# WdBlink/pyflyt-drone

Measured on AMD Instinct MI355X. Metric: env-steps/sec at N parallel envs (FixedwingWaypoints), higher is better.
Workload: dtype f64

## Files before the change

pyflyt-drone_amd/csrc/fwsim.hip:

```cpp
#include <hip/hip_runtime.h>

#include <algorithm>
#include <cmath>
#include <cstdio>
#include <cstdlib>
#include <cstring>
#include <map>
#include <mutex>
#include <new>
#include <string>
#include <type_traits>
#include <vector>

#include "fwsim_device.hpp"
#include "fwsim_rollout.hpp"
#include "fwsim_ppo.hpp"
#include "fwsim_collect.hpp"
#include "fwsim_fused.hpp"
#include "fwsim_objlock.hpp"
#include "fwsim_render.hpp"

using namespace fwsim;


// ... 87 lines not shown
  int left = (fresh && !begin) ? min(total - done, max_chunk > 0 ? max_chunk : P.step_ratio) : 0;
  if (__ballot(begin || left > 0) == 0ull) return;
  const DevState<T> V = shadow_view<T>(D);
  if (begin) {
    Rigid<T> S0; int32_t tick0 = 0, episode = (int32_t)target - 1, nr = 0; T wb0[3], wa0[3], wph0;
    T tm0[3]; (void)begin_reset<T, G>(P, V, env, S0, tick0, episode, nr, wb0, wa0, wph0, tm0);
    if (HASOBJ) {
      ObjState<T> O0;
      obj_reset_state<T, OBJ>(O0);
      if (OBJ) obj_spawn<T, G>(P, OC, V, env, target, leader, O0); else comb_spawn<T, G>(P, OC, V, env, target, leader, O0);
      if (leader) obj_store<T, OBJ>(V, env, O0);
    }
    if (leader) { store_rigid<T>(V, env, S0); D.is[env] = 0; D.sdone[env] = pack_done(target, D.epoch, sampled); }
  }
  if (__ballot(left > 0) == 0ull) return;
  TickC<T> C; SurfC<T> mine; T wmask;
  load_tick_constants<T, G, false>(Pp, C, mine, wmask);
  Rigid<T> S;
  load_rigid<T>(V, envc, S);
  T R[9];
  rot_from_unit_quat<T>(S.q, R);
  int32_t tick = D.is[envc];
  T wb[3], wa[3], wph;
#pragma unroll
  for (int k = 0; k < 3; ++k) { wb[k] = V.r[(RF_WIND + k) * n + envc]; wa[k] = V.r[(RF_WIND + 3 + k) * n + envc]; }
  wph = V.r[(RF_WIND + 6) * n + envc];
  T gust[2];
  gust_init<T>(P, wph, tick, gust);
  ObjState<T> O;
  if (HASOBJ) { obj_load<T, OBJ>(V, envc, O); O.near_mask = 0u; O.near_n = 0; }
  const T cmd0[FW_NUM_ACTUATORS] = {(T)0, (T)0, (T)0, (T)0, (T)0, (T)0};
  LaneAct<T> LA; LA.cmd = (T)0; LA.a = (T)0;
  if (G == 8) lane_act_scatter<T>(S, LA);
  const int chunk = left;
  int steps = sampled ? left : 0;
#pragma unroll 1
  while (__ballot(steps > 0) != 0ull) {
    const bool stepped = steps > 0;
    if (stepped) {
      (void)aviary_step<T, true, G, HASOBJ>(P, C, OC, V, envc, O, S, R, cmd0, tick, (T)0, (T)0, wb, wa, gust, mine, wmask, LA);
      steps -= 1;
    }
    if (HASOBJ) obj_capture_step<T, G>(OC, V, stepped, envc, O, S, R, tick);
  }
  if (G == 8) lane_act_gather<T>(S, LA);
  if (chunk > 0 && done + chunk == total) {
    T nd = (T)0;
    if (OBJ) obj_compute_state<T>(O);
    else {
      T t0[3];
#pragma unroll
      for (int k = 0; k < 3; ++k) t0[k] = V.r[(size_t)(RF_TARGETS + k) * n + envc];
      nd = end_reset<T, G>(P, V, envc, (int32_t)target, S, t0);
      if (COMB) comb_compute_state<T>(OC, O, P.num_targets == 0);
    }
    if (leader) {
      const T a0[4] = {(T)0, (T)0, (T)0, (T)0};
      T* orow = D.sobs + (size_t)env * P.obs_dim;
      if (OBJ) obj_write_obs<T>(P, O, S, a0, [&](int k, T v) { orow[k] = v; });
      else if (COMB) comb_write_obs<T>(P, V, env, O, S, a0, 0, [&](int k, T v) { orow[k] = v; });
      else write_obs<T>(P, V, env, S, a0, 0, [&](int k, T v) { orow[k] = v; });
      V.r[RF_NEW_DIST * n + env] = nd;
    }
  }
  if (chunk > 0 && leader) {
    store_rigid<T>(V, env, S);
    D.is[env] = tick;
    if (HASOBJ) obj_store<T, OBJ>(V, env, O);
    D.sdone[env] = pack_done(target, D.epoch, done + chunk);
  }
}

template <typename T, int G>
__device__ __forceinline__ void scenario_worker(const Params<T>* __restrict__ Pp, DevState<T> D, int blk) {
  constexpr int EPW = kWave / G;
  const int lane = threadIdx.x, sub = (G == 1) ? 0 : (lane & (G - 1)), row = lane / G;
  const int env = blk * EPW + row;
  const bool active = env < D.n;
  const int envc = active ? env : D.n - 1;
  const unsigned long long req = D.sreq[envc], dn = D.sdone[envc];
  const uint32_t target = (uint32_t)(req >> 32);
  const bool fresh = active && (uint32_t)req != D.epoch && req != ~0ull;
  const bool begin = fresh && (uint32_t)(dn >> 32) != target;
  if (__ballot(begin) == 0ull) return;
  if (begin) {
    const Params<T>& P = *Pp;
    Scenario<T> sc;
    sample_scenario_inl<T, G>(Pp, D.rs, (size_t)D.npad, env, target, &sc);
    T* orow = D.sobs + (size_t)env * P.obs_dim;
    for (int k = sub; k < P.att_dim; k += G) orow[k] = Pp->warm_obs[k];
    if (G > 1) {
      if (sub < P.ctx) {
        T d[3] = {(T)0, (T)0, (T)0}, b[3] = {(T)0, (T)0, (T)0};
        if (sub < P.num_targets) {
#pragma unroll
          for (int k = 0; k < 3; ++k) d[k] = sc.t_mine[k] - P.warm[k];
          mtv(P.warm_R, d, b);
        }
#pragma unroll
        for (int k = 0; k < 3; ++k) orow[P.att_dim + 3 * sub + k] = b[k];
      }
      if (sub == 0) {
        T nd = (T)0;
        if (P.num_targets > 0) {
          const T dx = sc.t_mine[0] - P.warm[0], dy = sc.t_mine[1] - P.warm[1], dz = sc.t_mine[2] - P.warm[2];
          nd = M<T>::sqrt_(dx * dx + dy * dy + dz * dz);
        }
        D.rs[(size_t)RF_NEW_DIST * D.npad + env] = nd;
      }
    }
    if (sub == 0) D.sdone[env] = pack_done(target, D.epoch, 1);
  }
}

#ifdef FW_PROFILE
#define FWP_NOW() ((long long)__builtin_readcyclecounter())
#define FWP(...) __VA_ARGS__
constexpr int kProfSlots = 256, kProfWords = 12;
#ifdef FW_PROFILE_PHASES
constexpr bool getenv_ph = true;
#else
constexpr bool getenv_ph = false;
#endif
#else
#define FWP(...)
#endif

enum Phase : int { PH_STEP = 0, PH_WARM = 1, PH_DONE = 2 };

template <typename T, bool GENERAL, int G, int TKIND, int WPE = 1, bool COLLECT = false, bool HELP = false, bool AX = false, bool AUX = false,
          typename SH = ShapeOfParams>
__device__ __forceinline__
void step_body(const Params<T>* __restrict__ Pp, const ObjC<T>* __restrict__ OCp, DevState<T> Dg,
               const T* __restrict__ actions, T* __restrict__ obs, T* __restrict__ reward,
               uint8_t* __restrict__ terminated, uint8_t* __restrict__ truncated, T* __restrict__ terminal_obs,
               int32_t* __restrict__ info, const CollectArgs* __restrict__ CAp = nullptr) {
  extern __shared__ __align__(16) unsigned char smem_raw[];
  T* tile = reinterpret_cast<T*>(smem_raw);
  const Params<T>& P = *Pp;
  constexpr bool OBJ = TKIND == FW_TASK_OBJLOCK;
  constexpr bool COMB = TKIND == FW_TASK_WAYPOINT_OBJLOCK;
  constexpr bool HASOBJ = OBJ || COMB;
  constexpr int EPW = kWave / G;
  constexpr bool DEFER = !GENERAL && TKIND == FW_TASK_WAYPOINTS;
  static_assert(!SH::kFixed || (std::is_same<T, double>::value && DEFER && G == 8 && !COLLECT && !HELP), "a fixed shape is threaded through the wind-free 8-lane waypoints path only");
  const int nblk = (Dg.npad + EPW - 1) / EPW;
  FWP(const long long p_t0 = FWP_NOW(); long long p_reset = 0, p_avi = 0, p_task = 0, p_r1 = 0, p_r2 = 0, p_r3 = 0; int p_nreset = 0, p_nhit = 0;)
  const int bx = (int)blockIdx.x - (COLLECT ? CAp->n_act : 0);
  const int wg = SH::kFixed ? (bx >= nblk ? bx - nblk : bx) : bx % nblk;
  const int blk = (G == 8 && (nblk & 7) == 0) ? (wg & 7) * (nblk >> 3) + (wg >> 3) : wg;
  const DevState<T> D = tile_view<T, EPW>(Dg, blk);
  if ((GENERAL || DEFER) && bx >= nblk) {
    if (AUX && threadIdx.x >= kWave) return;
    DevState<T> Dw = D;
    if constexpr (SH::kFixed) Dw.epoch = launch_index(Dg.lctr);
    if (GENERAL) shadow_worker<T, G, TKIND>(Pp, OCp, Dw, blk); else scenario_worker<T, G>(Pp, Dw, blk);
    FWP(if (D.prof && threadIdx.x == 0) {
      long long* w = D.prof + ((size_t)(Dw.epoch % kProfSlots) * 2 * nblk + blockIdx.x) * kProfWords;
      w[0] = FWP_NOW() - p_t0; })
    if constexpr (SH::kFixed) launch_done(Dg.lctr, Dw.epoch);
    return;
  }
  const int lane = AUX ? (int)(threadIdx.x & (kWave - 1)) : (int)threadIdx.x;
  const int sub = (G == 1) ? 0 : (lane & (G - 1));
  const int row = lane / G;
  const bool leader = sub == 0;
  const int env0 = blk * EPW;
  const int env = env0 + row;
  const bool active = env < D.n;
  const int envc = active ? env : D.n - 1;
  const size_t n = D.npad;
  const int Dobs = FW_SH(obs_dim);
  const int ld = Dobs + 1;

  T* aux_nz = AUX ? reinterpret_cast<T*>(smem_raw + Dg.mbox_off) : nullptr;
  if constexpr (AUX) {
    if (threadIdx.x >= kWave) {
      const int32_t a_tick = D.i[IF_TICK * n + envc], a_episode = D.i[IF_EPISODE * n + envc], a_flags = D.i[IF_FLAGS * n + envc];
      T a_z0 = (T)0, a_z1 = (T)0;
      if (FW_SH(has_noise) && FW_SH(step_ratio) <= G && !(a_flags & (FL_TERM | FL_TRUNC)))
        rng_normal2<T>(P, (uint32_t)(P.env_offset + envc), (uint32_t)a_episode, (uint32_t)(a_tick / FW_SH(ticks_per_aviary)) + (uint32_t)sub, a_z0, a_z1);
      aux_nz[2 * lane] = a_z0; aux_nz[2 * lane + 1] = a_z1;
      __syncthreads();
      return;
    }
  }

  int32_t step_count = D.i[IF_STEP * n + envc];
  int32_t tick = D.i[IF_TICK * n + envc];
  int32_t episode = D.i[IF_EPISODE * n + envc];
  int32_t flags = D.i[IF_FLAGS * n + envc];
  int32_t num_reached = D.i[IF_NUM_REACHED * n + envc];
  constexpr bool LANE_T = DEFER && G == 8;
  T tmine[3] = {(T)0, (T)0, (T)0};
  T a_keep = (T)0;
  if (LANE_T) {
    if (sub < FW_SH(num_targets)) {
#pragma unroll
      for (int k = 0; k < 3; ++k) tmine[k] = D.r[(size_t)(RF_TARGETS + 3 * sub + k) * n + envc];
    }
    if (!COLLECT) a_keep = actions[(size_t)envc * 4 + (sub & 3)];
  }
  Rigid<T> S;
  load_rigid<T>(D, envc, S);
  T new_dist = D.r[RF_NEW_DIST * n + envc];
  T ep_return = D.r[RF_EP_RETURN * n + envc];
  TickC<T> C; SurfC<T> mine_regs; T wmask;
  if constexpr (SH::kFixed) load_step_image<T>(Pp, C, mine_regs, wmask);
  else load_tick_constants<T, G, DEFER && G == 8 && WPE == 1>(Pp, C, mine_regs, wmask);
  uint32_t lctr_v = 0;
  if constexpr (SH::kFixed) lctr_v = vload(Dg.lctr + blockIdx.x + opaque_zero());
  if (AX && !SH::kFixed && sub >= FW_NUM_SURFACES) mine_regs.hra = (T)0;
  SurfC<T>& mine = mine_regs;

  normalize_quat<T>(S.q);
  T R[9];
  rot_from_unit_quat<T>(S.q, R);
  ObjState<T> O;
  const ObjC<T>& OC = *OCp;
  if (HASOBJ) { obj_load<T, OBJ>(D, envc, O); obj_update_near_mask<T, G>(P, OC, D, envc, O, S); }
  int32_t out_strike = 0;
  unsigned long long sh_req = ~0ull, sh_done = 0ull;
  if ((GENERAL || DEFER) && D.shadow_on) { sh_req = D.sreq[envc]; sh_done = D.sdone[envc]; }
  T wb[3] = {(T)0, (T)0, (T)0}, wa[3] = {(T)0, (T)0, (T)0}, wphase = (T)0;
  if (GENERAL) {
#pragma unroll
    for (int k = 0; k < 3; ++k) { wb[k] = D.r[(RF_WIND + k) * n + envc]; wa[k] = D.r[(RF_WIND + 3 + k) * n + envc]; }
    wphase = D.r[(RF_WIND + 6) * n + envc];
  }
  T gust[2] = {(T)0, (T)1};
  if (GENERAL) gust_init<T>(P, wphase, tick, gust);
  T rew = (T)-0.1;
  T cmd[FW_NUM_ACTUATORS];
  double c_ret = 0.0;
  if (COLLECT) {
    if (active && leader) c_ret = ld_sc1(CAp->S.returns + env);
    collect_wait_actions(*CAp, Dg.epoch, env0, min(EPW, Dg.n - env0));
  }
  {
    const T* ap = actions + (size_t)envc * 4;
    T a4[4];
    if (COLLECT) collect_load_actions<T>(*CAp, ap, a4);
    else {
#pragma unroll
      for (int k = 0; k < 4; ++k) a4[k] = ap[k];
    }
    if (COLLECT && LANE_T) a_keep = (sub & 3) == 0 ? a4[0] : (sub & 3) == 1 ? a4[1] : (sub & 3) == 2 ? a4[2] : a4[3];
    const T sp[4] = { a4[0], a4[1], a4[2], a4[3] * (T)0.5 + (T)0.5 };
#pragma unroll
    for (int c = 0; c < FW_NUM_ACTUATORS; ++c)
      cmd[c] = P.mixer[c][0] * sp[0] + P.mixer[c][1] * sp[1] + P.mixer[c][2] * sp[2] + P.mixer[c][3] * sp[3];
  }
  LaneAct<T> LA; LA.a = (T)0; LA.cmd = (T)0;
  T cmd_mine = (T)0;
  if (G == 8) { lane_act_scatter<T>(S, LA); cmd_mine = lane_pick5<T>(cmd[0], cmd[1], cmd[2], cmd[3], cmd[4]); LA.cmd = cmd_mine; }

  T tcur[3] = {(T)0, (T)0, (T)0}, tnext[3] = {(T)0, (T)0, (T)0};
  const int gbase = lane & ~(G - 1);
  if (LANE_T) {
#pragma unroll
    for (int k = 0; k < 3; ++k) tcur[k] = __shfl(tmine[k], gbase | (num_reached & (G - 1)), kWave);
  } else if (!OBJ) {
    const int i0 = min(num_reached, FW_MAX_TARGETS - 1), i1 = min(num_reached + 1, FW_MAX_TARGETS - 1);
#pragma unroll
    for (int k = 0; k < 3; ++k) {
      tcur[k] = D.r[(size_t)(RF_TARGETS + 3 * i0 + k) * n + envc];
      tnext[k] = D.r[(size_t)(RF_TARGETS + 3 * i1 + k) * n + envc];
    }
  }

  const uint32_t genv = (uint32_t)(P.env_offset + envc);
  const bool done_at_entry = (flags & (FL_TERM | FL_TRUNC)) != 0;
  int tgt_obs = (flags >> FL_TGT_SHIFT) & 15;
  flags &= FL_MASK;
  int act_src = done_at_entry ? 1 : 0;

  const uint32_t astep0 = (uint32_t)(tick / FW_SH(ticks_per_aviary));
  const bool pre_noise = (G == 8) && FW_SH(has_noise) && (FW_SH(step_ratio) <= G);
  T nz0 = (T)0, nz1 = (T)0;
  if (!AUX && pre_noise && !done_at_entry) rng_normal2<T>(P, genv, (uint32_t)episode, astep0 + (uint32_t)sub, nz0, nz1);

  int phase = active ? PH_STEP : PH_DONE;
  constexpr bool STASH = (!DEFER && !HASOBJ) || COLLECT;
  double* latch = STASH ? reinterpret_cast<double*>(smem_raw + Dg.stash_off) : nullptr;
  int it = 0, warm_left = 0;
  const Mbox<T> MB = mbox_at<T>(HELP ? Dg.mbox_off : 0);
  uint32_t n_posted = 0, pend_seq = 0;
  int pend = 0;
  T dist_keep = (T)0;
  bool resetting = false;
  bool step_over = active && done_at_entry;
  int32_t k_max_steps = 0, k_auto_reset = 0; T k_dome = (T)0, k_reach = (T)0;
  if constexpr (SH::kFixed) {
    k_max_steps = P.max_steps; k_auto_reset = P.auto_reset; k_dome = P.dome; k_reach = P.reach;
    asm("" : "+s"(k_max_steps)); asm("" : "+s"(k_auto_reset)); asm("" : "+s"(k_dome)); asm("" : "+s"(k_reach));
  }
  if constexpr (SH::kFixed) asm volatile("" : "+v"(lctr_v));
  if constexpr (AUX) {
    __syncthreads();
    nz0 = aux_nz[2 * lane]; nz1 = aux_nz[2 * lane + 1];
  }

  FWP(const long long p_t1 = FWP_NOW();)
#pragma unroll 1
  for (;;) {
    FWP(const long long p_a = FWP_NOW();)
    if (phase == PH_STEP && step_over) {
      step_count += 1;
      ep_return += rew;
      phase = PH_DONE;
      if (STASH && leader) {
        latch[4 * row] = (double)rew; latch[4 * row + 1] = (flags & (FL_TERM | FL_TRUNC)) ? 1.0 : 0.0;
        latch[4 * row + 2] = __hiloint2double(num_reached, flags); latch[4 * row + 3] = __hiloint2double(out_strike, step_count);
      }
      if (!(STASH && !DEFER) && leader) {
        reward[env] = rew;
        terminated[env] = (uint8_t)((flags & FL_TERM) ? 1 : 0);
        truncated[env] = (uint8_t)((flags & FL_TRUNC) ? 1 : 0);
        if (info) {
          int4* ip = reinterpret_cast<int4*>(info + (size_t)env * FW_INFO_DIM);
          ip[0] = make_int4(num_reached, (flags & FL_COLLISION) ? 1 : 0, (flags & FL_OOB) ? 1 : 0, (flags & FL_COMPLETE) ? 1 : 0);
          ip[1] = make_int4(out_strike, OBJ ? out_strike : 0, step_count, 0);
        }
      }
      if (DEFER) { resetting = (flags & (FL_TERM | FL_TRUNC)) && (SH::kFixed ? k_auto_reset : P.auto_reset); FWP(if (resetting) p_nreset += 1;) }
      const bool take_shadow = GENERAL && (flags & (FL_TERM | FL_TRUNC)) && P.auto_reset && D.shadow_on &&
                               (int)(sh_done & 0xFF) == P.warmup_aviary_steps + 1 && (uint32_t)(sh_done >> 32) == (uint32_t)(episode + 1) &&
                               (uint32_t)((sh_done >> 8) & 0xFFFFFFu) != (D.epoch & 0xFFFFFFu);
      if (take_shadow) { resetting = true; FWP(p_nreset += 1; p_nhit += 1;) }
      if (!DEFER && !take_shadow && (flags & (FL_TERM | FL_TRUNC)) && P.auto_reset) {
        if (G == 8) lane_act_gather<T>(S, LA);
        if (terminal_obs && leader) {
          T* trow = terminal_obs + (size_t)env * Dobs;
          T act_t[4];
          load_action<T, COLLECT>(D, actions, env, act_src, act_t);
          if (OBJ) obj_write_obs<T>(P, O, S, act_t, [&](int k, T v) { trow[k] = v; });
          else if (COMB) comb_write_obs<T>(P, D, env, O, S, act_t, tgt_obs, [&](int k, T v) { trow[k] = v; });
          else write_obs<T>(P, D, env, S, act_t, tgt_obs, [&](int k, T v) { trow[k] = v; });
        }
        T t_mine[3] = {(T)0, (T)0, (T)0};
        FWP(const long long p_ra = FWP_NOW(); p_r1 += p_ra - p_a;)
        {
          if (leader) stat_add(D.stats, FW_CTR_FALLBACKS);
          warm_left = begin_reset<T, G>(P, D, env, S, tick, episode, num_reached, wb, wa, wphase, t_mine);
          if (G > 1) {
            const int src = lane & ~(G - 1);
#pragma unroll
            for (int k = 0; k < 3; ++k) t_mine[k] = __shfl(t_mine[k], src, kWave);
          }
          if (HASOBJ) {
            obj_reset_state<T, OBJ>(O);
            if (OBJ) obj_spawn<T, G>(P, OC, D, env, (uint32_t)episode, leader, O);
            else comb_spawn<T, G>(P, OC, D, env, (uint32_t)episode, leader, O);
          }
        }
        if (G > 1 && warm_left > 0) __builtin_amdgcn_fence(__ATOMIC_ACQ_REL, "workgroup");
        if (HASOBJ) obj_update_near_mask<T, G>(P, OC, D, env, O, S);
        if (GENERAL) gust_init<T>(P, wphase, tick, gust);
        if (G == 8) lane_act_scatter<T>(S, LA);
        FWP(const long long p_rb = FWP_NOW(); p_r2 += p_rb - p_ra;)
        step_count = 0; flags = 0; ep_return = (T)0; tgt_obs = 0;
        act_src = 2;
        if (leader) stat_add(D.stats, FW_CTR_RESETS);
        FWP(p_nreset += 1;)
        rot_from_unit_quat<T>(S.q, R);
        if (GENERAL && warm_left > 0) phase = PH_WARM;
        else if (OBJ) obj_compute_state<T>(O);
        else {
          new_dist = end_reset<T, G>(P, D, env, episode, S, t_mine);
          if (COMB) comb_compute_state<T>(OC, O, P.num_targets == 0);
        }
        FWP(p_r3 += FWP_NOW() - p_rb;)
      }
    }
    FWP(const long long p_b = FWP_NOW(); p_reset += p_b - p_a;)
    if (__ballot(phase != PH_DONE) == 0ull) break;
    T z0 = (T)0, z1 = (T)0;
    if (pre_noise) {
      const int src = (lane & ~(G - 1)) | (it & (G - 1));
      z0 = __shfl(nz0, src, kWave); z1 = __shfl(nz1, src, kWave);
    }
    const bool stepped = phase != PH_DONE;
    const bool stepping = stepped && (!GENERAL || phase == PH_STEP);
    bool contact = false;
    if (stepped) {
      if (FW_SH(has_noise) && !pre_noise && stepping)
        rng_normal2<T>(P, genv, (uint32_t)episode, (uint32_t)(tick / FW_SH(ticks_per_aviary)), z0, z1);
      if (GENERAL) {
        T c_eff[FW_NUM_ACTUATORS];
#pragma unroll
        for (int c = 0; c < FW_NUM_ACTUATORS; ++c) c_eff[c] = stepping ? cmd[c] : (T)0;
        z0 = stepping ? z0 : (T)0; z1 = stepping ? z1 : (T)0;
        LA.cmd = stepping ? cmd_mine : (T)0;
        contact = aviary_step<T, true, G, HASOBJ, AX, SH>(P, C, OC, D, env, O, S, R, c_eff, tick, z0, z1, wb, wa, gust, mine, wmask, LA);
      } else {
        contact = aviary_step<T, false, G, HASOBJ, AX, SH>(P, C, OC, D, env, O, S, R, cmd, tick, z0, z1, wb, wa, gust, mine, wmask, LA);
      }
    }
    if constexpr (HELP) {
      const bool due = stepped && OC.camera_ratio_ticks > 0 && (tick % OC.camera_ratio_ticks) == 0;
      FWP(const long long p_c0 = FWP_NOW(); p_avi += p_c0 - p_b;)
      const uint32_t seq_cur = cap_post<T>(MB, n_posted, due, row, leader, O, S, R);
      FWP(p_r1 += FWP_NOW() - p_c0;)
      FWP(const long long p_w0 = FWP_NOW();)
      cap_collect<T>(MB, pend_seq, (pend & 2) != 0, row, O, D.stats);
      FWP(p_task += FWP_NOW() - p_w0;)
      pend_seq = 0;
      auto frame_half = [&](int keep) {
        if (OBJ) {
          obj_compute_state<T>(O);
          if ((keep & 4) && obj_reward<T>(OC, P.sparse, O, dist_keep, rew)) { flags |= FL_TERM | FL_COMPLETE; out_strike = 1; }
        } else {
          comb_compute_state<T>(OC, O, (keep & 8) != 0);
          if (keep & 4) {
            if (!(keep & 8)) comb_obstacle_penalty<T>(OC, O, (T)1, rew);
            else {
              comb_obstacle_penalty<T>(OC, O, (T)0.5, rew);
              if (comb_duck_reward<T>(OC, P.sparse, O, rew)) { flags |= FL_TERM | FL_COMPLETE; out_strike = 1; }
            }
          }
        }
      };
      FWP(const long long p_f0 = FWP_NOW();)
      if (pend & 1) frame_half(pend);
      FWP(const long long p_f1 = FWP_NOW(); p_r2 += p_f1 - p_f0;)
      pend = 0;
      int keep = 0;
      bool now = false;
      if (stepped) {
        if (stepping) {
          keep = 1 | (due ? 2 : 0);
          int nleft = 0;
          T old_dist = new_dist;
          if (COMB) {
            nleft = P.num_targets - num_reached;
            if (nleft > 0) {
              T dx = tcur[0] - S.p[0], dy = tcur[1] - S.p[1], dz = tcur[2] - S.p[2];
              new_dist = M<T>::sqrt_(dx * dx + dy * dy + dz * dz);
            }
            tgt_obs = num_reached;
            if (nleft == 0) keep |= 8;
          }
          if (step_count > P.max_steps) flags |= FL_TRUNC;
          if (contact) { rew = (T)-100; flags |= FL_COLLISION | FL_TERM; }
          if (S.p[0] * S.p[0] + S.p[1] * S.p[1] + S.p[2] * S.p[2] > P.dome * P.dome) { rew = (T)-100; flags |= FL_OOB | FL_TERM; }
          bool can_strike = false;
          if (!(flags & (FL_COLLISION | FL_OOB))) {
            keep |= 4;
            if (OBJ) {
              T dx = O.duck[0] - S.p[0], dy = O.duck[1] - S.p[1], dz = O.duck[2] - S.p[2];
              dist_keep = M<T>::sqrt_(dx * dx + dy * dy + dz * dz);
              can_strike = O.lock_steps + (T)1 >= (T)OC.hold_steps && dist_keep <= OC.strike_dist;
            } else if (nleft > 0) {
              if (!P.sparse) {
                T progress = (old_dist != (T)0) ? (old_dist - new_dist) : (T)0;
                rew += M<T>::fmax_((T)3 * progress, (T)0);
                rew += M<T>::rcp_(new_dist);
              }
              if (new_dist < P.reach) {
                rew = (T)100;
                num_reached += 1;
                if (num_reached == P.num_targets) flags &= ~(FL_TERM | FL_TRUNC);
                const int i1 = min(num_reached + 1, FW_MAX_TARGETS - 1);
#pragma unroll
                for (int k = 0; k < 3; ++k) { tcur[k] = tnext[k]; tnext[k] = D.r[(size_t)(RF_TARGETS + 3 * i1 + k) * n + env]; }
              }
            } else {
              flags &= ~FL_TERM;
              can_strike = O.lock_steps + (T)1 >= (T)OC.hold_steps;
            }
          }
          step_over = (it + 1 >= P.step_ratio) || (flags & (FL_TERM | FL_TRUNC));
          now = can_strike || step_over;
        } else {
          now = true;
        }
      }
      auto finish_now = [&]() {
        if (stepping) {
          frame_half(keep);
          step_over = (it + 1 >= P.step_ratio) || (flags & (FL_TERM | FL_TRUNC));
        } else {
          warm_left -= 1;
          if (warm_left == 0) {
            if (OBJ) obj_compute_state<T>(O);
            else { new_dist = end_reset<T, G>(P, D, env, episode, S); comb_compute_state<T>(OC, O, P.num_targets == 0); }
            phase = PH_DONE;
          }
        }
      };
      FWP(const long long p_f2 = FWP_NOW(); p_r3 += p_f2 - p_f1;)
      bool wait_here;
      if constexpr (OBJ) wait_here = __ballot(now && due) != 0ull; else wait_here = __ballot(now) != 0ull;
      if (wait_here) {
        FWP(const long long p_w1 = FWP_NOW();)
        cap_collect<T>(MB, seq_cur, due, row, O, D.stats);
        FWP(p_task += FWP_NOW() - p_w1; p_nhit += 1;)
        FWP(const long long p_f3 = FWP_NOW();)
        if (stepped) finish_now();
        FWP(p_r2 += FWP_NOW() - p_f3;)
      } else {
        FWP(const long long p_f3 = FWP_NOW();)
        if constexpr (OBJ) { if (now) finish_now(); else pend = keep; }
        else pend = keep;
        FWP(p_r2 += FWP_NOW() - p_f3;)
        pend_seq = seq_cur;
      }
    } else {
    if (HASOBJ) obj_capture_step<T, G, COLLECT>(OC, D, stepped, envc, O, S, R, tick);
    FWP(const long long p_c = FWP_NOW(); p_avi += p_c - p_b;)
    if (stepped) {
      if (stepping && OBJ) {
        obj_compute_state<T>(O);
        if (step_count > P.max_steps) flags |= FL_TRUNC;
        if (contact) { rew = (T)-100; flags |= FL_COLLISION | FL_TERM; }
        if (S.p[0] * S.p[0] + S.p[1] * S.p[1] + S.p[2] * S.p[2] > P.dome * P.dome) { rew = (T)-100; flags |= FL_OOB | FL_TERM; }
        if (!(flags & (FL_COLLISION | FL_OOB))) {
          T dx = O.duck[0] - S.p[0], dy = O.duck[1] - S.p[1], dz = O.duck[2] - S.p[2];
          if (obj_reward<T>(OC, P.sparse, O, M<T>::sqrt_(dx * dx + dy * dy + dz * dz), rew)) {
            flags |= FL_TERM | FL_COMPLETE; out_strike = 1;
          }
        }
        step_over = (it + 1 >= P.step_ratio) || (flags & (FL_TERM | FL_TRUNC));
      } else if (stepping && COMB) {
        const int nleft = P.num_targets - num_reached;
        const T old_dist = new_dist;
        if (nleft > 0) {
          T dx = tcur[0] - S.p[0], dy = tcur[1] - S.p[1], dz = tcur[2] - S.p[2];
          new_dist = M<T>::sqrt_(dx * dx + dy * dy + dz * dz);
        }
        tgt_obs = num_reached;
        comb_compute_state<T>(OC, O, nleft == 0);
        if (step_count > P.max_steps) flags |= FL_TRUNC;
        if (contact) { rew = (T)-100; flags |= FL_COLLISION | FL_TERM; }
        if (S.p[0] * S.p[0] + S.p[1] * S.p[1] + S.p[2] * S.p[2] > P.dome * P.dome) { rew = (T)-100; flags |= FL_OOB | FL_TERM; }
        if (!(flags & (FL_COLLISION | FL_OOB))) {
          if (nleft > 0) {
            if (!P.sparse) {
              T progress = (old_dist != (T)0) ? (old_dist - new_dist) : (T)0;
              rew += M<T>::fmax_((T)3 * progress, (T)0);
              rew += M<T>::rcp_(new_dist);
            }
            if (new_dist < P.reach) {
              rew = (T)100;
              num_reached += 1;
              if (num_reached == P.num_targets) flags &= ~(FL_TERM | FL_TRUNC);
              const int i1 = min(num_reached + 1, FW_MAX_TARGETS - 1);
#pragma unroll
              for (int k = 0; k < 3; ++k) { tcur[k] = tnext[k]; tnext[k] = D.r[(size_t)(RF_TARGETS + 3 * i1 + k) * n + env]; }
            }
            comb_obstacle_penalty<T>(OC, O, (T)1, rew);
          } else {
            flags &= ~FL_TERM;
            comb_obstacle_penalty<T>(OC, O, (T)0.5, rew);
            if (comb_duck_reward<T>(OC, P.sparse, O, rew)) { flags |= FL_TERM | FL_COMPLETE; out_strike = 1; }
          }
        }
        step_over = (it + 1 >= P.step_ratio) || (flags & (FL_TERM | FL_TRUNC));
      } else if (stepping) {
        const int nleft = FW_SH(num_targets) - num_reached;
        const T old_dist = new_dist;
        if (FW_SH(task) != FW_TASK_OBJLOCK && nleft > 0) {
          T dx = tcur[0] - S.p[0], dy = tcur[1] - S.p[1], dz = tcur[2] - S.p[2];
          if constexpr (SH::kFixed) new_dist = M<T>::sqrt_(sum_squares_fma(dx, dy, dz));
          else new_dist = M<T>::sqrt_(dx * dx + dy * dy + dz * dz);
        }
        tgt_obs = num_reached;
        if (step_count > (SH::kFixed ? k_max_steps : P.max_steps)) flags |= FL_TRUNC;
        if (contact) { rew = (T)-100; flags |= FL_COLLISION | FL_TERM; }
        bool oob;
        if constexpr (SH::kFixed) oob = sum_squares_fma(S.p[0], S.p[1], S.p[2]) > k_dome * k_dome;
        else oob = S.p[0] * S.p[0] + S.p[1] * S.p[1] + S.p[2] * S.p[2] > P.dome * P.dome;
        if (oob) { rew = (T)-100; flags |= FL_OOB | FL_TERM; }
        if (FW_SH(task) != FW_TASK_OBJLOCK && nleft > 0) {
          if (!FW_SH(sparse)) {
            T progress = (old_dist != (T)0) ? (old_dist - new_dist) : (T)0;
            rew += M<T>::fmax_((T)3 * progress, (T)0);
            rew += M<T>::rcp_(new_dist);
          }
          if (new_dist < (SH::kFixed ? k_reach : P.reach)) {
            rew = (T)100;
            num_reached += 1;
            if (num_reached == FW_SH(num_targets)) flags |= FL_TRUNC | FL_COMPLETE;
            if (LANE_T) {
#pragma unroll
              for (int k = 0; k < 3; ++k) tcur[k] = __shfl(tmine[k], gbase | (num_reached & (G - 1)), kWave);
            } else {
              const int i1 = min(num_reached + 1, FW_MAX_TARGETS - 1);
#pragma unroll
              for (int k = 0; k < 3; ++k) { tcur[k] = tnext[k]; tnext[k] = D.r[(size_t)(RF_TARGETS + 3 * i1 + k) * n + env]; }
            }
          }
        }
        step_over = (it + 1 >= FW_SH(step_ratio)) || (flags & (FL_TERM | FL_TRUNC));
      } else {
        warm_left -= 1;
        if (warm_left == 0) {
          if (OBJ) obj_compute_state<T>(O);
          else { new_dist = end_reset<T, G>(P, D, env, episode, S); if (COMB) comb_compute_state<T>(OC, O, P.num_targets == 0); }
          phase = PH_DONE;
        }
      }
      FWP(p_task += FWP_NOW() - p_c;)
    }
    }
    it += 1;
  }
  FWP(const long long p_t2 = FWP_NOW();)
  if (G > 1 && !DEFER) __builtin_amdgcn_fence(__ATOMIC_ACQ_REL, "workgroup");
  if (G == 8) lane_act_gather<T>(S, LA);
  T tpre[3] = {(T)0, (T)0, (T)0};
  const uint32_t launch = SH::kFixed ? 1u + (uint32_t)__builtin_amdgcn_readfirstlane((int)lctr_v) : D.epoch;
  const bool pre = DEFER && resetting && D.shadow_on && (int)(sh_done & 0xFF) == 1 && (uint32_t)(sh_done >> 32) == (uint32_t)(episode + 1) &&
                   (uint32_t)((sh_done >> 8) & 0xFFFFFFu) != (launch & 0xFFFFFFu);
  if (pre) {
#pragma unroll
    for (int k = 0; k < 3; ++k) pf_issue(tpre[k], &D.rs[(size_t)(RF_TARGETS + 3 * sub + k) * n + env]);
  }
  constexpr bool WO = DEFER && G == 8;
  constexpr int kWO = WO ? 32 / G : 1;
  T wo[kWO];
  if (WO && resetting) {
#pragma unroll
    for (int j = 0; j < kWO; ++j) { const int k = sub + j * G; wo[j] = (k < FW_SH(att_dim)) ? vload(&Pp->warm_obs[k]) : (T)0; }
  }

  constexpr int kDOW = 4;
  T dow[kDOW], dnd = (T)0;
  if (WO && pre && Dobs <= kDOW * G) {
#pragma unroll
    for (int j = 0; j < kDOW; ++j) { const int k = sub + j * G; dow[j] = (T)0; if (k < Dobs) pf_issue(dow[j], &Dg.sobs[(size_t)env * Dobs + k]); }
    pf_issue(dnd, &D.rs[(size_t)RF_NEW_DIST * n + env]);
  }

  constexpr int kRows = HASOBJ ? RF_COUNT : RF_TASK;
  constexpr int kCW = GENERAL ? (kRows + G - 1) / G : 1, kOW = GENERAL ? (kMaxObs + G - 1) / G : 1;
  constexpr bool SWAP_REGS = GENERAL && G == 8;
  T cw[kCW], ow[kOW];
  int32_t tick_new = 0;
  constexpr bool PF_GEN = false;
  if (GENERAL && resetting) {
    if (SWAP_REGS) {
#pragma unroll
      for (int j = 0; j < kCW; ++j) {
        const int w = sub + j * G; cw[j] = (T)0;
        if (w < kRows) { if (PF_GEN) pf_issue(cw[j], &D.rs[(size_t)w * n + env]); else cw[j] = D.rs[(size_t)w * n + env]; }
      }
#pragma unroll
      for (int j = 0; j < kOW; ++j) {
        const int k = sub + j * G; ow[j] = (T)0;
        if (k < Dobs) { if (PF_GEN) pf_issue(ow[j], &Dg.sobs[(size_t)env * Dobs + k]); else ow[j] = Dg.sobs[(size_t)env * Dobs + k]; }
      }
    }
    tick_new = D.is[env];
  }
  const int ep_want = episode + 1 + ((GENERAL && resetting) ? 1 : 0);
  if ((GENERAL || DEFER) && D.shadow_on && active && leader && (uint32_t)(sh_req >> 32) != (uint32_t)ep_want)
    D.sreq[env] = ((unsigned long long)(uint32_t)ep_want << 32) | (unsigned long long)launch;
  T act_obs[4] = {(T)0, (T)0, (T)0, (T)0};
  if (LANE_T) {
#pragma unroll
    for (int k = 0; k < 4; ++k) act_obs[k] = __shfl(a_keep, gbase | k, kWave);
    if (act_src == 1) {
#pragma unroll
      for (int k = 0; k < 4; ++k) act_obs[k] = D.r[(size_t)(RF_ACTION + k) * n + envc];
    }
    T Ro[9];
    int o = write_obs_attitude<T, true, SH>(P, S, act_obs, Ro, [&](int k, T v) { if (leader) tile[row * ld + k] = v; });
#pragma unroll SH::kCtxUnroll
    for (int i = 0; i < FW_SH(ctx); ++i) {
      const int t = tgt_obs + i;
      T tw[3], d[3], b[3] = {(T)0, (T)0, (T)0};
#pragma unroll
      for (int k = 0; k < 3; ++k) tw[k] = __shfl(tmine[k], gbase | (t & (G - 1)), kWave);
      if (t < FW_SH(num_targets)) {
#pragma unroll
        for (int k = 0; k < 3; ++k) d[k] = tw[k] - S.p[k];
        mtv(Ro, d, b);
      }
      if (leader) { tile[row * ld + o] = b[0]; tile[row * ld + o + 1] = b[1]; tile[row * ld + o + 2] = b[2]; }
      o += 3;
    }
  } else if (active && leader) {
    load_action<T, COLLECT>(D, actions, env, act_src, act_obs);
    if (OBJ) obj_write_obs<T>(P, O, S, act_obs, [&](int k, T v) { tile[row * ld + k] = v; });
    else if (COMB) comb_write_obs<T>(P, D, env, O, S, act_obs, tgt_obs, [&](int k, T v) { tile[row * ld + k] = v; });
    else write_obs<T>(P, D, env, S, act_obs, tgt_obs, [&](int k, T v) { tile[row * ld + k] = v; });
  }
  FWP(const long long p_e0 = FWP_NOW();)
  if (DEFER && pre) {
    pf_wait(tpre[0], tpre[1], tpre[2], dnd);
    if (WO) pf_tie(dow[0], dow[1], dow[2], dow[3]);
  }
  if (DEFER && resetting) {
    __builtin_amdgcn_fence(__ATOMIC_ACQ_REL, "wavefront");
    if (terminal_obs) {
      T* trow = terminal_obs + (size_t)env * Dobs;
      for (int k = sub; k < Dobs; k += G) trow[k] = tile[row * ld + k];
    }
    __builtin_amdgcn_fence(__ATOMIC_ACQ_REL, "wavefront");
    FWP(const long long p_e1 = FWP_NOW(); p_r1 = p_e1 - p_e0;)
    episode += 1;
    if (leader) { stat_add(D.stats, FW_CTR_RESETS); stat_add(D.stats, pre ? FW_CTR_SCENARIO_HITS : FW_CTR_FALLBACKS); }
    Scenario<T> sc;
    if (pre) {
#pragma unroll
      for (int k = 0; k < 3; ++k) sc.t_mine[k] = tpre[k];
      if (sub < FW_SH(num_targets)) {
#pragma unroll
        for (int k = 0; k < 3; ++k) D.r[(size_t)(RF_TARGETS + 3 * sub + k) * n + env] = tpre[k];
      }
    } else {
      sample_scenario_inl<T, G>(Pp, D.r, n, env, (uint32_t)episode, &sc);
    }
    const int nt = min(FW_SH(ctx), FW_SH(num_targets));
    T t0[3] = {(T)0, (T)0, (T)0};
    const bool copied = WO && pre && Dobs <= kDOW * G;
    if (copied) {
#pragma unroll
      for (int j = 0; j < kDOW; ++j) { const int k = sub + j * G; if (k < Dobs) tile[row * ld + k] = dow[j]; }
    }
#pragma unroll 1
    for (int i = 0; i < (copied ? 0 : FW_SH(ctx)); ++i) {
      T tw[3] = {(T)0, (T)0, (T)0};
      if (G > 1) {
#pragma unroll
        for (int k = 0; k < 3; ++k) tw[k] = __shfl(sc.t_mine[k], (lane & ~(G - 1)) | (i & (G - 1)), kWave);
      } else if (i < nt) {
#pragma unroll
        for (int k = 0; k < 3; ++k) tw[k] = D.r[(size_t)(RF_TARGETS + 3 * i + k) * n + env];
      }
      T d[3] = {(T)0, (T)0, (T)0}, b[3] = {(T)0, (T)0, (T)0};
      if (i < nt) {
#pragma unroll
        for (int k = 0; k < 3; ++k) d[k] = tw[k] - P.warm[k];
        mtv(P.warm_R, d, b);
        if (i == 0) { t0[0] = tw[0]; t0[1] = tw[1]; t0[2] = tw[2]; }
      }
      if (leader) { tile[row * ld + FW_SH(att_dim) + 3 * i] = b[0]; tile[row * ld + FW_SH(att_dim) + 3 * i + 1] = b[1]; tile[row * ld + FW_SH(att_dim) + 3 * i + 2] = b[2]; }
    }
    FWP(const long long p_e2 = FWP_NOW(); p_r2 = p_e2 - p_e1;)
    if (WO && !copied) {
#pragma unroll
      for (int j = 0; j < kWO; ++j) { const int k = sub + j * G; if (k < FW_SH(att_dim)) tile[row * ld + k] = wo[j]; }
    }
    if (!copied) for (int k = sub + (WO ? kWO * G : 0); k < FW_SH(att_dim); k += G) tile[row * ld + k] = Pp->warm_obs[k];
#pragma unroll
    for (int k = 0; k < 3; ++k) { S.p[k] = P.warm[k]; S.v[k] = P.warm[7 + k]; S.w[k] = P.warm[10 + k]; }
#pragma unroll
    for (int k = 0; k < 4; ++k) S.q[k] = P.warm[3 + k];
#pragma unroll
    for (int k = 0; k < FW_NUM_ACTUATORS; ++k) S.act[k] = P.warm[13 + k];
    tick = P.warm_ticks;
    step_count = 0; flags = 0; ep_return = (T)0; tgt_obs = 0; num_reached = 0;
    new_dist = copied ? dnd : (T)0;
    if (FW_SH(num_targets) > 0 && !copied) {
      if (G == 1 && nt == 0) {
#pragma unroll
        for (int k = 0; k < 3; ++k) t0[k] = D.r[(size_t)(RF_TARGETS + k) * n + env];
      } else if (G > 1 && nt == 0) {
#pragma unroll
        for (int k = 0; k < 3; ++k) t0[k] = __shfl(sc.t_mine[k], lane & ~(G - 1), kWave);
      }
      T dx = t0[0] - S.p[0], dy = t0[1] - S.p[1], dz = t0[2] - S.p[2];
      new_dist = M<T>::sqrt_(dx * dx + dy * dy + dz * dz);
    }
#pragma unroll
    for (int k = 0; k < 4; ++k) act_obs[k] = (T)0;
    FWP(p_r3 = FWP_NOW() - p_e2;)
  }
  if (PF_GEN && resetting) {
    asm volatile("s_waitcnt vmcnt(0)" ::: "memory");
#pragma unroll
    for (int j = 0; j < kCW; ++j) asm volatile("" : "+v"(cw[j]));
#pragma unroll
    for (int j = 0; j < kOW; ++j) asm volatile("" : "+v"(ow[j]));
  }
  if (GENERAL && resetting) {
    __builtin_amdgcn_fence(__ATOMIC_ACQ_REL, "wavefront");
    if (terminal_obs) {
      T* trow = terminal_obs + (size_t)env * Dobs;
      for (int k = sub; k < Dobs; k += G) trow[k] = tile[row * ld + k];
    }
    __builtin_amdgcn_fence(__ATOMIC_ACQ_REL, "wavefront");
    if (SWAP_REGS) {
#pragma unroll
      for (int j = 0; j < kOW; ++j) { const int k = sub + j * G; if (k < Dobs) tile[row * ld + k] = ow[j]; }
#pragma unroll
      for (int j = 0; j < kCW; ++j) { const int w = sub + j * G; if (w < kRows) D.r[(size_t)w * n + env] = cw[j]; }
    } else {
      for (int k = 0; k < Dobs; ++k) tile[row * ld + k] = Dg.sobs[(size_t)env * Dobs + k];
      copy_words<T, G>(D.r, D.rs, 0, kRows, n, env);
    }
    if (leader) { stat_add(D.stats, FW_CTR_RESETS); stat_add(D.stats, FW_CTR_SHADOW_HITS); }
    episode += 1; tick = tick_new;
    step_count = 0; flags = 0; tgt_obs = 0; num_reached = 0;
  }
  if (active && leader) {
    if (!(GENERAL && resetting)) {
      store_rigid<T>(D, env, S);
      if (HASOBJ) obj_store<T, OBJ>(D, env, O);
#pragma unroll
      for (int k = 0; k < 4; ++k) D.r[(RF_ACTION + k) * n + env] = act_obs[k];
      D.r[RF_NEW_DIST * n + env] = new_dist;
      D.r[RF_EP_RETURN * n + env] = ep_return;
    }
    D.i[IF_STEP * n + env] = step_count;
    D.i[IF_TICK * n + env] = tick;
    D.i[IF_EPISODE * n + env] = episode;
    D.i[IF_FLAGS * n + env] = flags | (tgt_obs << FL_TGT_SHIFT);
    D.i[IF_NUM_REACHED * n + env] = num_reached;
  }
  if (STASH && !DEFER && active && leader) {
    const double w2 = latch[4 * row + 2], w3 = latch[4 * row + 3];
    const int o_nr = __double2hiint(w2), o_fl = __double2loint(w2), o_st = __double2hiint(w3), o_sc = __double2loint(w3);
    reward[env] = (T)latch[4 * row];
    terminated[env] = (uint8_t)((o_fl & FL_TERM) ? 1 : 0);
    truncated[env] = (uint8_t)((o_fl & FL_TRUNC) ? 1 : 0);
    if (info) {
      int4* ip = reinterpret_cast<int4*>(info + (size_t)env * FW_INFO_DIM);
      ip[0] = make_int4(o_nr, (o_fl & FL_COLLISION) ? 1 : 0, (o_fl & FL_OOB) ? 1 : 0, (o_fl & FL_COMPLETE) ? 1 : 0);
      ip[1] = make_int4(o_st, OBJ ? o_st : 0, o_sc, 0);
    }
  }
  if (HELP || AUX) { __builtin_amdgcn_fence(__ATOMIC_ACQ_REL, "workgroup"); __builtin_amdgcn_wave_barrier(); }
  else __syncthreads();
  if (COLLECT) collect_stats_tail<T>(*CAp, D.epoch, tile, ld, min(EPW, D.n - env0), wg, nblk, active && leader, latch[4 * row], latch[4 * row + 1] != 0.0, env, c_ret);
  flush_obs_tile<T>(tile, ld, obs, env0, EPW, D.n, Dobs);
  if (COLLECT && active && leader) collect_clear_actions<T>(const_cast<T*>(actions) + (size_t)env * 4);
  FWP(long long p_capmax = HASOBJ ? O.p_cap : 0; const int p_ncapw = HASOBJ ? __popcll(__ballot(leader && O.p_ncap > 0)) : 0;)
  FWP(if (D.prof) {
    for (int o = 32; o > 0; o >>= 1) p_capmax = max(p_capmax, (long long)__shfl_xor((long long)p_capmax, o, kWave));
    const int nr = __popcll(__ballot(leader && p_nreset > 0)), nh = __popcll(__ballot(leader && p_nhit > 0));
    for (int o = 32; o > 0; o >>= 1) {
      p_r1 = max(p_r1, (long long)__shfl_xor((long long)p_r1, o, kWave));
      p_r2 = max(p_r2, (long long)__shfl_xor((long long)p_r2, o, kWave));
      p_r3 = max(p_r3, (long long)__shfl_xor((long long)p_r3, o, kWave));
    }
    if (lane == 0) {
      long long* w = D.prof + ((size_t)(launch % kProfSlots) * 2 * nblk + blockIdx.x) * kProfWords;
      const long long t3 = FWP_NOW();
      w[0] = t3 - p_t0; w[1] = p_t1 - p_t0; w[2] = p_reset; w[3] = p_avi; w[4] = p_task; w[5] = t3 - p_t2; w[6] = it | (nr << 8) | (nh << 16); w[7] = p_t0; w[8] = p_r1; w[9] = p_r2; w[10] = p_r3;
      w[11] = p_capmax | ((long long)p_ncapw << 48);
      if (HELP) { w[8] = p_nhit; w[9] = n_posted; w[7] = p_r1; w[10] = p_r2; w[11] = p_r3; }
      else if (HASOBJ) { w[8] = O.p_capm[0]; w[9] = O.p_capm[1]; w[10] = O.p_capm[2]; w[7] = O.p_capm[3];
        if (getenv_ph) { w[1] = O.p_ph[0]; w[3] = O.p_ph[1]; w[4] = O.p_ph[2]; w[5] = O.p_ph[3]; w[9] = O.p_ph[4]; w[6] = O.p_ph[5]; } }
    } })
  if constexpr (SH::kFixed) launch_done(Dg.lctr, launch);
}

#ifndef FW_G1_WAVES
#define FW_G1_WAVES 2
#endif
#define FW_STEP_ARGS const Params<T>* __restrict__ Pp, const ObjC<T>* __restrict__ OCp, DevState<T> D,                  \
    const T* __restrict__ actions, T* __restrict__ obs, T* __restrict__ reward, uint8_t* __restrict__ terminated,        \
    uint8_t* __restrict__ truncated, T* __restrict__ terminal_obs, int32_t* __restrict__ info
#define FW_STEP_PASS Pp, OCp, D, actions, obs, reward, terminated, truncated, terminal_obs, info
#define FW_STEP_RUN(...) do { D.epoch = launch_index(D.lctr); step_body<__VA_ARGS__>(FW_STEP_PASS); launch_done(D.lctr, D.epoch); } while (0)
template <typename T, bool GENERAL, bool AX = false>
__global__ __launch_bounds__(kWave) void fw_step_kernel_g8(FW_STEP_ARGS) { FW_STEP_RUN(T, GENERAL, 8, FW_TASK_WAYPOINTS, 1, false, false, AX); }
template <typename T>
__global__ __launch_bounds__(2 * kWave) void fw_step_kernel_g8x(FW_STEP_ARGS) { FW_STEP_RUN(T, false, 8, FW_TASK_WAYPOINTS, 1, false, false, true, true); }
template <typename T>
__global__ __launch_bounds__(2 * kWave) void fw_step_kernel_g8xs(FW_STEP_ARGS) {
  step_body<T, false, 8, FW_TASK_WAYPOINTS, 1, false, false, true, true, ShapeTrainWaypoints>(FW_STEP_PASS);
}
template <typename T, bool GENERAL>
__global__ __launch_bounds__(kWave) __attribute__((amdgpu_waves_per_eu(2, 2)))
void fw_step_kernel_g8w2(FW_STEP_ARGS) { FW_STEP_RUN(T, GENERAL, 8, FW_TASK_WAYPOINTS, 2); }
template <typename T, bool GENERAL>
__global__ __launch_bounds__(kWave) __attribute__((amdgpu_waves_per_eu(FW_G1_WAVES, FW_G1_WAVES)))
void fw_step_kernel_g1(FW_STEP_ARGS) { FW_STEP_RUN(T, GENERAL, 1, FW_TASK_WAYPOINTS); }
template <typename T, int TKIND>
__global__ __launch_bounds__(kWave) void fw_step_kernel_obj_g8(FW_STEP_ARGS) { FW_STEP_RUN(T, true, 8, TKIND); }
template <typename T, int TKIND>
__global__ __launch_bounds__(kWave) void fw_step_kernel_obj_g1(FW_STEP_ARGS) { FW_STEP_RUN(T, true, 1, TKIND); }
#ifndef FW_HELP_CHUNK
#define FW_HELP_CHUNK 2
#endif
template <typename T, int TKIND>
__global__ __launch_bounds__(2 * kWave) void fw_step_kernel_obj_g8h(FW_STEP_ARGS) {
  const Mbox<T> MB = mbox_at<T>(D.mbox_off);
  if (threadIdx.x < 4) MB.ctl[threadIdx.x] = 0u;
  __syncthreads();
  if (threadIdx.x >= kWave) {
    const int nblk = (D.npad + 7) / 8, bx = (int)blockIdx.x % nblk;
    const int blk = ((nblk & 7) == 0) ? (bx & 7) * (nblk >> 3) + (bx >> 3) : bx;
    D.epoch = launch_index(D.lctr);
    const DevState<T> V = tile_view<T, 8>(D, blk);
    FWP(const long long h0 = FWP_NOW(); long long hcap = 0; int hreq = 0;)
    if (D.shadow_on) shadow_worker<T, 8, TKIND>(Pp, OCp, V, blk, FW_HELP_CHUNK);
    FWP(const long long h1 = FWP_NOW();)
    capture_server<T>(MB, 0u, *OCp, V, blk * 8 FWP(, &hcap, &hreq));
    FWP(if (D.prof && threadIdx.x == kWave) {
      long long* w = D.prof + ((size_t)(D.epoch % kProfSlots) * 2 * nblk + nblk + blockIdx.x) * kProfWords;
      w[0] = (h1 - h0) + hcap; w[1] = h1 - h0; w[2] = hcap; w[3] = hreq; w[4] = FWP_NOW() - h0; })
    return;
  }
  D.epoch = launch_index(D.lctr);
  step_body<T, true, 8, TKIND, 1, false, true>(FW_STEP_PASS);
  launch_done(D.lctr, D.epoch);
  if (threadIdx.x == 0) __hip_atomic_store(MB.ctl + 2, 1u, __ATOMIC_RELEASE, __HIP_MEMORY_SCOPE_WORKGROUP);
}

#define FW_COLLECT_RUN(T_, ...) do {                                                                                       \
    if ((int)blockIdx.x < CA.n_act) {                                                                                  \
       \
      const int nblk_ = (D.npad + 7) / 8, c_ = min((int)blockIdx.x >> 1, CA.n_chunks - 1);                              \
      const int blk_ = min(c_ * kCRows / 8, nblk_ - 1);                                                                 \
      const int wg_ = ((nblk_ & 7) == 0) ? (blk_ % (nblk_ >> 3)) * 8 + blk_ / (nblk_ >> 3) : blk_;    \
// ... 2190 lines not shown
```

Before: 256.1 million.

## Add specialized fixed-shape step loop replacing phase state machine

For the compile-time fixed-shape specialization, replaces the general phase-driven for(;;) state machine with a straight counted loop over step_ratio physics substeps. Reward, termination and target advancement are computed inline, and the episode outcome is written once after the loop. This removes per-iteration phase dispatch and divergence, and the loop exits early via a ballot once no lane is still stepping. It skips the in-loop reset and warm-up paths and the STASH/DEFER latch handling for this specialization, so it relies on those being handled elsewhere or not used with fixed shapes.

```diff
diff --git a/pyflyt-drone_amd/csrc/fwsim.hip b/pyflyt-drone_amd/csrc/fwsim.hip
--- a/pyflyt-drone_amd/csrc/fwsim.hip
+++ b/pyflyt-drone_amd/csrc/fwsim.hip
@@ -413,6 +413,65 @@
   }
 
   FWP(const long long p_t1 = FWP_NOW();)
+  if constexpr (SH::kFixed) {
+    bool stepping = active && !done_at_entry;
+#pragma unroll 1
+    for (it = 0; it < SH::step_ratio; ++it) {
+      FWP(const long long p_b = FWP_NOW();)
+      if (__ballot(stepping) == 0ull) break;
+      const int src = (lane & ~(G - 1)) | (it & (G - 1));
+      const T z0 = __shfl(nz0, src, kWave), z1 = __shfl(nz1, src, kWave);
+      bool contact = false;
+      if (stepping) contact = aviary_step<T, false, G, false, AX, SH>(P, C, OC, D, env, O, S, R, cmd, tick, z0, z1, wb, wa, gust, mine, wmask, LA);
+      FWP(const long long p_c = FWP_NOW(); p_avi += p_c - p_b;)
+      if (stepping) {
+        const int nleft = SH::num_targets - num_reached;
+        const T old_dist = new_dist;
+        if (nleft > 0) {
+          T dx = tcur[0] - S.p[0], dy = tcur[1] - S.p[1], dz = tcur[2] - S.p[2];
+          new_dist = M<T>::sqrt_(sum_squares_fma(dx, dy, dz));
+        }
+        tgt_obs = num_reached;
+        if (step_count > k_max_steps) flags |= FL_TRUNC;
+        if (contact) { rew = (T)-100; flags |= FL_COLLISION | FL_TERM; }
+        if (sum_squares_fma(S.p[0], S.p[1], S.p[2]) > k_dome * k_dome) { rew = (T)-100; flags |= FL_OOB | FL_TERM; }
+        if (nleft > 0) {
+          if (!SH::sparse) {
+            T progress = (old_dist != (T)0) ? (old_dist - new_dist) : (T)0;
+            rew += M<T>::fmax_((T)3 * progress, (T)0);
+            rew += M<T>::rcp_(new_dist);
+          }
+          if (new_dist < k_reach) {
+            rew = (T)100;
+            num_reached += 1;
+            if (num_reached == SH::num_targets) flags |= FL_TRUNC | FL_COMPLETE;
+#pragma unroll
+            for (int k = 0; k < 3; ++k) tcur[k] = __shfl(tmine[k], gbase | (num_reached & (G - 1)), kWave);
+          }
+        }
+        if (flags & (FL_TERM | FL_TRUNC)) stepping = false;
+        FWP(p_task += FWP_NOW() - p_c;)
+      }
+    }
+    FWP(const long long p_a = FWP_NOW();)
+    if (active) {
+      step_count += 1;
+      ep_return += rew;
+      if (leader) {
+        reward[env] = rew;
+        terminated[env] = (uint8_t)((flags & FL_TERM) ? 1 : 0);
+        truncated[env] = (uint8_t)((flags & FL_TRUNC) ? 1 : 0);
+        if (info) {
+          int4* ip = reinterpret_cast<int4*>(info + (size_t)env * FW_INFO_DIM);
+          ip[0] = make_int4(num_reached, (flags & FL_COLLISION) ? 1 : 0, (flags & FL_OOB) ? 1 : 0, (flags & FL_COMPLETE) ? 1 : 0);
+          ip[1] = make_int4(out_strike, 0, step_count, 0);
+        }
+      }
+      resetting = (flags & (FL_TERM | FL_TRUNC)) && k_auto_reset;
+      FWP(if (resetting) p_nreset += 1;)
+    }
+    FWP(p_reset += FWP_NOW() - p_a;)
+  } else {
 #pragma unroll 1
   for (;;) {
     FWP(const long long p_a = FWP_NOW();)
@@ -717,6 +776,7 @@
     }
     it += 1;
   }
+  }
   FWP(const long long p_t2 = FWP_NOW();)
   if (G > 1 && !DEFER) __builtin_amdgcn_fence(__ATOMIC_ACQ_REL, "workgroup");
   if (G == 8) lane_act_gather<T>(S, LA);
```

Result: faster. 274.3 million (median of 6 runs) (+7.1%).
